# microsoft/EVA

Hardware: AMD Instinct MI355X
Metric: homomorphic ops/sec (mul+rescale+relin) at N=2^16, L=10; execute() wall-time (higher is better)
Workload: dtype u64

## Files before the change

### eva_amd/backend.py

```python
import ctypes as C
import os

import numpy as np

from . import _hipruntime

_HERE = os.path.dirname(os.path.abspath(__file__))
LIB_PATH = os.path.join(_HERE, "lib", "libeva_hip.so")

KEY_RELIN = 0
KEY_GALOIS = 1
F64, F32, U8 = 0, 1, 2
_DTYPES = {np.dtype(np.float64): F64, np.dtype(np.float32): F32, np.dtype(np.uint8): U8}


def array_dtype(a):
    a = np.asarray(a)
    if a.dtype not in _DTYPES or not a.flags["C_CONTIGUOUS"]:
        a = np.ascontiguousarray(a, dtype=np.float64)
    return a, _DTYPES[a.dtype]


class EvaHipError(RuntimeError):
    pass
# ... 8 lines not shown
    "evah_ctx_create": [C.c_uint32, C.c_uint32, _u64p, C.c_int, _vpp],
    "evah_ctx_fork": [_vp, _vpp],
    "evah_ctx_set_stream": [_vp, _vp],
    "evah_ctx_sync": [_vp],
    "evah_ctx_mem_info": [_vp, C.POINTER(C.c_size_t), C.POINTER(C.c_size_t)],
    "evah_key_upload": [_vp, C.c_int, C.c_uint32, C.c_uint32, _u64p],
    "evah_galois_elt_from_step": [_vp, C.c_int32, C.POINTER(C.c_uint32)],
    "evah_ct_upload": [_vp, C.c_uint32, C.c_uint32, C.c_double, _u64p, _vpp],
    "evah_ct_write": [_vp, _vp, _u64p],
    "evah_ct_copy": [_vp, _vp, _vpp],
    "evah_ct_assign": [_vp, _vp, _vp],
    "evah_ctx_wait": [_vp, _vp],
    "evah_ctx_transfer_stats": [_vp, _u64p],
    "evah_ctx_modup_variant": [_vp, C.POINTER(C.c_uint32)],
    "evah_ctx_tail_variant": [_vp, C.POINTER(C.c_uint32)],
    "evah_ctx_key_bytes": [_vp, _u64p],
    "evah_ctx_key_bytes_detail": [_vp, _u64p],
    "evah_ctx_key_upload_stats": [_vp, _u64p],
    "evah_pt_copy": [_vp, _vp, _vpp],
    "evah_pt_write": [_vp, _vp, _u64p],
    "evah_capture_begin": [_vp, _vpp, C.c_uint32],
    "evah_capture_end": [_vp, _vpp, C.c_uint32, _vpp],
    "evah_graph_launch": [_vp, _vp],
    "evah_ct_info": [_vp, C.POINTER(C.c_uint32), C.POINTER(C.c_uint32), C.POINTER(C.c_double)],
    "evah_ct_download": [_vp, _vp, _u64p],
    "evah_pt_upload": [_vp, C.c_uint32, C.c_double, _u64p, _vpp],
    "evah_pt_upload_coeff": [_vp, C.c_uint32, C.c_double, _u64p, _vpp],
    "evah_pt_uniform": [_vp, C.c_uint32, C.c_double, _u64p, _vpp],
    "evah_pt_info": [_vp, C.POINTER(C.c_uint32), C.POINTER(C.c_double)],
    "evah_pt_download": [_vp, _vp, _u64p],
# ... 639 lines not shown
    def transfer_stats(self):
        out = (C.c_uint64 * 6)()
        _chk(_lib.evah_ctx_transfer_stats(self.h, out))
        return tuple(int(x) for x in out)

    def modup_variant(self):
        out = (C.c_uint32 * 3)()
        _chk(_lib.evah_ctx_modup_variant(self.h, out))
        return int(out[0]), bool(out[1]), bool(out[2])

    def tail_variant(self):
        out = (C.c_uint32 * 3)()
        _chk(_lib.evah_ctx_tail_variant(self.h, out))
        return bool(out[0]), bool(out[1]), bool(out[2])

    def key_bytes(self):
        out = C.c_uint64()
        _chk(_lib.evah_ctx_key_bytes(self.h, C.byref(out)))
        return int(out.value)

    def key_bytes_detail(self):
        out = (C.c_uint64 * 3)()
        _chk(_lib.evah_ctx_key_bytes_detail(self.h, out))
        return tuple(int(x) for x in out)

    def key_upload_stats(self):
        out = (C.c_uint64 * 2)()
        _chk(_lib.evah_ctx_key_upload_stats(self.h, out))
        return tuple(int(x) for x in out)

# ... 376 lines not shown
```

### eva_amd/csrc/internal.hip.h

```cpp
#pragma once
#include "../../include/eva_hip.h"

#include <hip/hip_runtime.h>

#include <algorithm>
#include <cmath>
#include <cstdlib>
#include <cstring>
#include <functional>
#include <map>
#include <memory>
#include <mutex>
#include <stdexcept>
#include <string>
#include <tuple>
#include <unordered_map>
#include <vector>

#include "devmath.hip.h"
#include "hostmath.h"

namespace evah {

extern thread_local std::string g_err;
// ... 183 lines not shown
  bool fold_pa = true;
  bool win_fuse = true;
  bool win_linear = true;
  bool fb_persist = true;
  uint32_t fb_grid = 0;
  bool mac3 = true;
  uint32_t loop_n = 8, loop_min = 2, loop_min_wgs = 2048, loop_target_wgs = 8192;
  bool hoist_map = true;
  bool side_stream = false;
  bool chain_step = true, chain_batched = true;
  uint32_t chain_fuse_blocks = 256;
  bool modup = true;
  int modup_lr = 3;
  bool modup_spec = true;
  bool tail_fuse = true;
  uint32_t lds_extra = 0;
  uint32_t keygen_set_words = 1u << 27;

  static Tunables from_env(uint32_t N) {
    Tunables t;
    auto flag = [](const char *name, bool &v) { if (const char *e = std::getenv(name)) v = std::atoi(e) != 0; };
    auto count = [](const char *name, uint32_t &v) { if (const char *e = std::getenv(name)) v = (uint32_t)std::max(0, std::atoi(e)); };
    (void)N;
    flag("EVAH_FUSE_MAC", t.fuse_mac);
    flag("EVAH_FUSE_MUL", t.fuse_mul);
    flag("EVAH_FUSE_MUL2", t.fuse_mul2);
    flag("EVAH_EW_FUSE", t.ew_fuse);
    flag("EVAH_EW_UNIFORM", t.ew_uniform);
    count("EVAH_FUSE_SMALL", t.fuse_small_blocks);
    if (const char *e = std::getenv("EVAH_SMALL_LR")) t.small_lr = std::atoi(e) == 3 ? 3 : 2;
// ... 13 lines not shown
    count("EVAH_LOOP_N", t.loop_n);
    count("EVAH_LOOP_MIN", t.loop_min);
    count("EVAH_LOOP_MIN_WGS", t.loop_min_wgs);
    count("EVAH_LOOP_TARGET_WGS", t.loop_target_wgs);
    count("EVAH_LDS_EXTRA", t.lds_extra);
    count("EVAH_KEYGEN_SET_WORDS", t.keygen_set_words);
    flag("EVAH_HOIST_MAP", t.hoist_map);
    flag("EVAH_SIDE_STREAM", t.side_stream);
    flag("EVAH_CHAIN_STEP", t.chain_step);
    flag("EVAH_CHAIN_BATCHED", t.chain_batched);
    count("EVAH_CHAIN_FUSE_BLOCKS", t.chain_fuse_blocks);
    flag("EVAH_MODUP", t.modup);
    if (const char *e = std::getenv("EVAH_MODUP_LR")) t.modup_lr = std::atoi(e) == 2 ? 2 : 3;
    flag("EVAH_MODUP_SPEC", t.modup_spec);
    flag("EVAH_TAIL_FUSE", t.tail_fuse);
    if (const char *e = std::getenv("EVAH_KS_GROUPS")) t.ks_groups = std::max(1, std::atoi(e));
    if (const char *e = std::getenv("EVAH_KS_THREADS")) {
      const int n = std::atoi(e);
      if (n == 64 || n == 128 || n == 256) t.ks_threads = n;
    }
    return t;
  }
};

struct evah_ctx {
  std::shared_ptr<SharedDev> sh;
  int device = 0;
  uint32_t N = 0, logN = 0, k = 0;
  std::vector<u64> primes;
  std::vector<int> total_bits;
// ... 25 lines not shown

#ifndef EVAH_TOPBIT
#define EVAH_TOPBIT 1
#endif
struct ModupVariant { int lr; bool tbonly, lazyonly; };
inline ModupVariant modup_variant(const evah_ctx *c) {
  const bool tb = c->tun.modup_spec && EVAH_TOPBIT && c->modup_tb;
  return {c->tun.modup_lr, tb, tb && c->modup_lazy};
}
struct TailVariant { bool fused, tbonly, lazyonly; };
inline TailVariant tail_variant(const evah_ctx *c) {
  const bool tb = c->tun.modup_spec && EVAH_TOPBIT && c->modup_tb;
  return {c->tun.tail_fuse, tb, tb && c->tail_lazy};
}

inline void use(evah_ctx *c) { HIPCHK(hipSetDevice(c->device)); }
inline void count_h2d(evah_ctx *c, size_t bytes, bool plain = false) { c->sh->xfer[plain ? 2 : 0]++; c->sh->xfer[4] += bytes; }
inline void count_d2h(evah_ctx *c, size_t bytes, bool plain = false) { c->sh->xfer[plain ? 3 : 1]++; c->sh->xfer[5] += bytes; }

inline hipEvent_t prof_event(evah_ctx *c) {
  if (!c->prof_free.empty()) {
    hipEvent_t e = c->prof_free.back();
    c->prof_free.pop_back();
    return e;
  }
  hipEvent_t e;
  HIPCHK(hipEventCreate(&e));
  return e;
}
inline void prof_drain(evah_ctx *c) {
// ... 259 lines not shown
```

### eva_amd/csrc/keyswitch.hip

```cpp
#include "launch.hip.h"

namespace evah {

__global__ void __launch_bounds__(256)
k_ks_mac(DevCtx cx, const u64 *target, const u64 *scratch, const u64 *key, u64 *prod, uint32_t l) {
  if (cx.skipped()) return;
  const uint32_t I = blockIdx.y;
  const uint32_t kap = (I == l) ? cx.k - 1 : I;
  const size_t n = 2 * ((size_t)blockIdx.x * blockDim.x + threadIdx.x);
  const DevPrime pm = cx.primes[kap];
  const size_t N = cx.N, key_digit = (size_t)2 * cx.k * N;
  u128_t a0x = {0, 0}, a0y = {0, 0}, a1x = {0, 0}, a1y = {0, 0};
  for (uint32_t J = 0; J < l; J++) {
    const u64 *op = (I == J) ? target + (size_t)J * N : scratch + ((size_t)I * l + J) * N;
    const ulonglong2 o = ld2(op + n);
    const u64 *kp = key + J * key_digit + (size_t)kap * N + n;
    const ulonglong2 k0 = ld2(kp), k1 = ld2(kp + (size_t)cx.k * N);
    acc128(a0x, o.x, k0.x);
    acc128(a0y, o.y, k0.y);
    acc128(a1x, o.x, k1.x);
    acc128(a1y, o.y, k1.y);
  }
  ulonglong2 r0, r1;
  r0.x = barrett128(a0x, pm);
// ... 24 lines not shown
  return kb;
}

template <int P>
static void launch_ks_inner_p(evah_ctx *c, const u64 *target, const u64 *scratch, const KsBatch &kb, u64 *prod, uint32_t l) {
  constexpr int LR = KS_LR;
  ProfScope ps(c, KC_KSMAC);
  const uint32_t tile = ks_wg_threads(c) << LR;
  const bool one_wave = ks_one_wave(c);
  const int logC = (int)ilog2(tile) - P;
  if (logC < 0) throw std::runtime_error("ks_inner tile smaller than one sub-transform");
  const size_t lds = ((((size_t)1 << logC) * lds_sub_stride<P>() + 1) & ~(size_t)1) * sizeof(u64) +
                     ((size_t)1 << (logC + P)) * sizeof(ulonglong2) +
                     (kb.mac3 ? (size_t)tile * sizeof(u64) : 0);
  const uint32_t n_tiles = c->N / tile;
  auto go = [&](auto kernel, const auto &mt, const auto &at) {
    hipLaunchKernelGGL(kernel, dim3(n_tiles * kb.n, kb.ni), dim3(tile >> LR), lds, c->stream, c->dev, target, kb.target_bs, scratch,
                       kb.scratch_bs, kb.keys, prod, kb.prod_bs, l, kb.i0, logC, n_tiles, kb.n, kb.targets, mt, kb.istep,
                       kb.nout ? kb.nout : l + 1, kb.r_out, at, (kb.lazy_out ? 1 : 0) | (kb.diag ? 2 : 0), kb.fold_row);
  };
  if (kb.r_out && (!one_wave || kb.istep != 1)) throw std::logic_error("fused special-row inverse pass needs the one-wave key-switch kernel");
  if (kb.fold && kb.istep != 1) throw std::logic_error("the folded key-switch forms are not used on limb shards");
  if (kb.fold && !kb.mul && !kb.adds) throw std::logic_error("folded key switch without polynomials to fold");
  const int mode = kb.mul ? (kb.fold ? KS_FOLDMUL : KS_MUL) : (kb.fold ? KS_FOLDADD : KS_PLAIN);
  auto with_mode = [&](auto mode_tag) {
    constexpr int M = decltype(mode_tag)::value;
    const KsMulArg<M> mt = [&] { if constexpr (M == KS_MUL || M == KS_FOLDMUL) return *kb.mul; else return NoMul{}; }();
    const KsAddArg<M> at = [&] { if constexpr (M == KS_FOLDADD) return *kb.adds; else return NoMul{}; }();
    if constexpr (M != KS_MUL) {
      if (kb.mac3 && one_wave) {
        if (kb.r_out) go(ks_inner_kernel<P, LR, 64, M, true, true>, mt, at);
        else go(ks_inner_kernel<P, LR, 64, M, false, true>, mt, at);
        return;
      }
    }
    if (kb.mac3) throw std::logic_error("split keys handed to a key-switch kernel that accumulates in 128 bits");
    if (kb.r_out) go(ks_inner_kernel<P, LR, 64, M, true>, mt, at);
    else if (one_wave) go(ks_inner_kernel<P, LR, 64, M>, mt, at);
    else go(ks_inner_kernel<P, LR, NTT_THREADS, M>, mt, at);
  };
  switch (mode) {
  case KS_PLAIN: with_mode(std::integral_constant<int, KS_PLAIN>{}); break;
  case KS_MUL: with_mode(std::integral_constant<int, KS_MUL>{}); break;
// ... 7 lines not shown
  case 5: launch_ks_inner_p<5>(c, target, scratch, key, prod, l); break;
  case 6: launch_ks_inner_p<6>(c, target, scratch, key, prod, l); break;
  case 7: launch_ks_inner_p<7>(c, target, scratch, key, prod, l); break;
  case 8: launch_ks_inner_p<8>(c, target, scratch, key, prod, l); break;
  default: throw std::runtime_error("unsupported poly_modulus_degree for the key-switch kernel");
  }
}

static bool ks_small(evah_ctx *c, uint32_t l, uint32_t n) {
  return c->tun.fuse_mac && std::max(1, c->tun.ks_groups) == 1 && fuse_small_launch(c, n * (l + 1) * l);
}
static bool ks_takes_modup(evah_ctx *c, uint32_t l, uint32_t n) {
  return !ks_small(c, l, n) && c->tun.modup && c->tun.fuse_mac && std::max(1, c->tun.ks_groups) == 1 && modup_fits(c);
}

bool switch_key_products(evah_ctx *c, uint32_t l, const u64 *target, size_t target_bs, const KeyDev *const *keys,
                         uint32_t n, u64 *prod_d, const PtrTab *target_tab, const MulTab *mul, u64 *r_small, bool fold,
                         const PtrTab *adds, bool lazy_out) {
  const size_t N = c->N;
  KsBatch kb = ks_batch(c, l, keys, n, !(mul && !fold));
  kb.target_bs = target_bs;
  if (target_tab) kb.targets = *target_tab;
  kb.mul = mul;
  kb.fold = fold;
  kb.adds = adds;
  kb.lazy_out = lazy_out;
  if ((mul || fold) && !c->tun.fuse_mac) throw std::logic_error("the fused multiply / folded forms need the fused key-switch kernel");
  Scratch t(c, (size_t)n * l * N);
  Scratch sc(c, n * kb.scratch_bs);
  Scratch d2(c, mul && fold ? (size_t)n * l * N : 1);
  if (mul && fold) {
    target = d2.d;
    kb.target_bs = target_bs = (size_t)l * N;
  }
  OpKsDigit::Params dp{t.d, sc.d, l, (size_t)l * N, kb.scratch_bs, 0, l + 1};
// ... 9 lines not shown
    if (small || modup) launch_pass_p<false, true, OpPlain>(c, c->logN / 2, ip, n * l);
    else ntt_inverse<OpPlain>(c, ip, n * l);
  }
  if (small) {
    dp.i0 = kb.i0 = 0;
    dp.ni = kb.ni = l + 1;
    launch_inv_fwd<OpKsDigit>(c, dp, n * (l + 1) * l);
    if (r_small && c->tun.fuse_special_inv && ks_one_wave(c)) kb.r_out = r_small;
    launch_ks_inner(c, c->logN / 2, target, sc.d, kb, prod_d, l);
    return kb.r_out != nullptr;
  }
  if (c->tun.fuse_mac) {
    const int a = (c->logN + 1) / 2, b = c->logN / 2;
    const uint32_t groups = std::min<uint32_t>(std::max(1, c->tun.ks_groups), l + 1);
    if (r_small && groups == 1 && c->tun.fuse_special_inv && ks_one_wave(c)) kb.r_out = r_small;
    for (uint32_t g = 0; g < groups; g++) {
      const uint32_t i0 = (uint32_t)((uint64_t)(l + 1) * g / groups), i1 = (uint32_t)((uint64_t)(l + 1) * (g + 1) / groups);
      if (i1 == i0) continue;
      dp.i0 = kb.i0 = i0;
      dp.ni = kb.ni = i1 - i0;
      if (modup) launch_modup<OpKsDigit>(c, dp, n);
      else launch_pass_p<true, false, OpKsDigit>(c, a, dp, n * (i1 - i0) * l);
      launch_ks_inner(c, b, target, sc.d, kb, prod_d, l);
    }
    return kb.r_out != nullptr;
  } else {
    ntt_forward<OpKsDigit>(c, dp, n * (l + 1) * l);
    for (uint32_t b = 0; b < n; b++) {
      ProfScope ps(c, KC_KSMAC);
      hipLaunchKernelGGL(k_ks_mac, dim3(c->N / 512, l + 1), dim3(256), 0, c->stream, c->dev,
// ... 62 lines not shown
  OpModDown::Params mp{r.d, N, prod.d, pps, nullptr, 0, 0, out_d, (size_t)l * N, c->k - 1, l};
  mp.use_add_tab = !fold;
  mp.add_tab = in.c01;
  inverse_then_forward<OpPlain, OpModDown>(c, sp, 2 * n, mp, 2 * n * l, inv1);
}

static void relin_rescale_core(evah_ctx *c, uint32_t l, uint32_t n, const Size3Tab *in, const MulTab *mul, u64 *out_d) {
  const uint32_t last = l - 1, sp = c->k - 1;
  const size_t N = c->N, pps = (size_t)(l + 1) * N, ops = (size_t)(l - 1) * N;
  PtrTab c2{}, a_last{}, a_polys{};
  if (in) {
    c2 = in->c2;
    a_polys = in->c01;
    for (uint32_t i = 0; i < 2 * n; i++) a_last.p[i] = a_polys.p[i] + (size_t)last * N;
  }
  Scratch prod(c, (size_t)n * 2 * pps);
  std::vector<const KeyDev *> keys(n, &c->sh->relin);
  const bool fold = c->tun.fold_pa && c->tun.fuse_mac;
  switch_key_products(c, l, nullptr, 0, keys.data(), n, prod.d, &c2, mul, nullptr, fold, mul ? nullptr : &a_polys, fold);
  Scratch r(c, (size_t)n * 2 * N), t(c, (size_t)n * 2 * N);
  if (fold && tail_variant(c).fused && ks_takes_modup(c, l, n)) {
    OpRRLastFolded::Params lp{nullptr, 0, prod.d + (size_t)last * N, pps, r.d, N, t.d, N, last, sp, {}};
    OpTailIntt::Params ip{lp, prod.d + (size_t)l * N, pps, r.d};
    launch_pass_p<false, true, OpTailIntt>(c, c->logN / 2, ip, 4 * n);
    OpRRFolded::Params rp{r.d, N, t.d, N, nullptr, 0, prod.d, pps, out_d, ops, sp, last, l - 1, {}};
    launch_tail(c, lp, rp, 2 * n);
    launch_pass_p<false, false, OpRRFolded>(c, c->logN / 2, rp, 2 * n * (l - 1));
    return;
  }
  OpPlain::Params spp{prod.d + (size_t)l * N, r.d, pps, N, 1, sp, 1, {}};
  ntt_inverse<OpPlain>(c, spp, 2 * n);
  if (fold) {
    OpRRLastFolded::Params lp{nullptr, 0, prod.d + (size_t)last * N, pps, r.d, N, t.d, N, last, sp, {}};
// ... 335 lines not shown
```

### eva_amd/csrc/launch.hip.h

```cpp
#pragma once
#include "internal.hip.h"
#include "ntt.hip.h"

namespace evah {

#define EW_SETUP                                                                                 \
  const uint32_t p = blockIdx.z, i = blockIdx.y;                                                 \
  const size_t off = (size_t)i * cx.N + 2 * ((size_t)blockIdx.x * blockDim.x + threadIdx.x);    \
  const DevPrime pm = cx.primes[cx.prime_of(i)];                                                 \
  (void)p;                                                                                        \
  (void)pm;

__device__ __forceinline__ ulonglong2 ld2(const u64 *p) { return *reinterpret_cast<const ulonglong2 *>(p); }
__device__ __forceinline__ void st2(u64 *p, ulonglong2 v) { *reinterpret_cast<ulonglong2 *>(p) = v; }
__device__ __forceinline__ u64 split30(u64 k) { return (k & 0x3fffffffull) | ((k >> 30) << 32); }

template <class Op> struct OpClass;
template <bool Z, bool G> struct OpClass<OpPlainT<Z, G>> { static constexpr int fwd_a = KC_NTT_A, fwd_b = KC_NTT_B; };
template <> struct OpClass<OpMulIntt> { static constexpr int fwd_a = KC_NTT_A, fwd_b = KC_NTT_B; };
template <> struct OpClass<OpKsDigit> { static constexpr int fwd_a = KC_KSDIGIT_A, fwd_b = KC_KSDIGIT_B; };
template <bool G> struct OpClass<OpModDownT<G>> { static constexpr int fwd_a = KC_MODDOWN_A, fwd_b = KC_MODDOWN_B; };
template <> struct OpClass<OpMulPolyIntt> { static constexpr int fwd_a = KC_NTT_A, fwd_b = KC_NTT_B; };
template <> struct OpClass<OpModDownMul> { static constexpr int fwd_a = KC_MODDOWN_A, fwd_b = KC_MODDOWN_B; };
template <int M> struct OpClass<OpRRT<M>> { static constexpr int fwd_a = KC_MODDOWN_A, fwd_b = KC_MODDOWN_B; };
// ... 91 lines not shown
struct KsBatch {
  uint32_t n = 1;
  uint32_t i0 = 0, ni = 0;
  size_t target_bs = 0, scratch_bs = 0, prod_bs = 0;
  KsKeys keys{};
  PtrTab targets{};
  const MulTab *mul = nullptr;
  bool fold = false;
  const PtrTab *adds = nullptr;
  bool mac3 = false;
  bool lazy_out = false;
  uint32_t istep = 1, nout = 0;
  u64 *r_out = nullptr;
  bool diag = false;
  uint32_t fold_row = ~0u;
};
inline std::vector<double> fill_mul_tab(evah_ctx *c, const evah_ct *const *as, const evah_ct *const *bs, uint32_t pairs, uint32_t B,
                                        uint32_t l, const char *batch_msg, MulTab &tab) {
  std::vector<double> scales(pairs);
  for (uint32_t i = 0; i < pairs; i++) {
    const evah_ct *a = as[i], *b = bs[i];
    if (a->size != 2 || b->size != 2) throw std::invalid_argument("multiply supports size-2 operands only (relinearize first)");
    if (a->batch != B || b->batch != B) throw std::invalid_argument(batch_msg);
    if (a->limbs != l || b->limbs != l) throw std::invalid_argument("encrypted parameter mismatch in batch");
    scales[i] = a->scale * b->scale;
    check_scale(c, scales[i], l);
    acquire(c, a->buf);
    acquire(c, b->buf);
    for (uint32_t x = 0; x < B; x++) {
      tab.a[i * B + x] = a->d + (size_t)x * 2 * a->ps;
// ... 135 lines not shown
static void inverse_then_forward(evah_ctx *c, const typename InvOp::Params &ip, uint32_t inv_jobs, const typename Op::Params &fp,
                                 uint32_t fwd_jobs, bool inv_pass1_done = false) {
  if (inv_pass1_done && !fuse_small_launch(c, fwd_jobs)) throw std::logic_error("fused inverse pass outside the small-launch form");
  if (fuse_small_launch(c, fwd_jobs)) {
    if (!inv_pass1_done) launch_pass_p<false, true, InvOp>(c, c->logN / 2, ip, inv_jobs);
    launch_inv_fwd<Op>(c, fp, fwd_jobs);
    launch_pass_p<false, false, Op>(c, c->logN / 2, fp, fwd_jobs);
  } else {
    ntt_inverse<InvOp>(c, ip, inv_jobs);
    ntt_forward<Op>(c, fp, fwd_jobs);
  }
}

bool switch_key_products(evah_ctx *c, uint32_t l, const u64 *target, size_t target_bs, const KeyDev *const *keys, uint32_t n,
                         u64 *prod_d, const PtrTab *target_tab = nullptr, const MulTab *mul = nullptr, u64 *r_small = nullptr,
                         bool fold = false, const PtrTab *adds = nullptr, bool lazy_out = false);
void switch_key(evah_ctx *c, uint32_t l, const u64 *target, const KeyDev &key, const u64 *add, size_t add_ps, uint32_t add_polys,
                u64 *out, size_t out_ps);
void key_split_launch(evah_ctx *c, const u64 *src, u64 *dst, size_t words);
const uint32_t *perm_table(evah_ctx *c, uint32_t elt);
void galois_perm_launch(evah_ctx *c, const u64 *a, size_t a_ps, uint32_t limbs, uint32_t polys, const uint32_t *perm, u64 *out, size_t o_ps);
void enc_tables(evah_ctx *c);

}
```

### eva_amd/csrc/ntt_ks_inner.hip.h

```cpp
#pragma once
#include "ntt.hip.h"

namespace evah {

#ifndef EVAH_KS_BATCH_MAX_DEFINED
#define EVAH_KS_BATCH_MAX_DEFINED
constexpr int KS_BATCH_MAX = 64;
#endif
struct KsKeys {
  const u64 *key[KS_BATCH_MAX];
  uint32_t rows;
};
struct PtrTab {
  const u64 *p[2 * KS_BATCH_MAX];
};

struct MulTab {
  const u64 *a[KS_BATCH_MAX], *b[KS_BATCH_MAX];
  uint32_t a_ps[KS_BATCH_MAX], b_ps[KS_BATCH_MAX];
};
struct MulSrc {
  const u64 *a, *b;
  size_t sa, sb;
};
// ... 34 lines not shown
  s2 = mad64(v1, (uint32_t)(kw >> 32), s2);
}
__device__ __forceinline__ void mac3_fold(u64 &s0, u64 &s1, u64 &s2) {
  s1 += s0 >> 30;
  s0 &= 0x3fffffffull;
  s2 += s1 >> 30;
  s1 &= 0x3fffffffull;
}
__device__ __forceinline__ u128_t mac3_recombine(u64 s0, u64 s1, u64 s2) {
  unsigned __int128 a = s0;
  a += (unsigned __int128)s1 << 30;
  a += (unsigned __int128)s2 << 60;
  return {(u64)a, (u64)(a >> 64)};
}

template <int P, int LR, int MAXT, int MODE, bool INVSP = false, bool MAC3 = false>
__global__ void __launch_bounds__(MAXT)
ks_inner_kernel(DevCtx cx, const u64 *__restrict__ target_b, size_t target_bs, const u64 *__restrict__ scratch_b,
                size_t scratch_bs, KsKeys keys, u64 *__restrict__ prod_b, size_t prod_bs, uint32_t l, uint32_t i0,
                int logC, uint32_t n_tiles, uint32_t n_inst, PtrTab targets, KsMulArg<MODE> mul, uint32_t istep,
                uint32_t nout, u64 *__restrict__ r_out, KsAddArg<MODE> adds, int flags, uint32_t fold_row) {
  const bool lazy_out = flags & 1, diag = flags & 2;
  constexpr bool MUL = MODE == KS_MUL;
  extern __shared__ __attribute__((aligned(16))) u64 lds[];
  if (cx.skipped()) return;
  uint32_t tile_idx, inst;
  if ((n_tiles & 7u) == 0) {
    const uint32_t x = blockIdx.x, lo = x & 7u, rest = x >> 3;
    inst = rest % n_inst;
    tile_idx = (rest / n_inst) * 8u + lo;
  } else {
    inst = blockIdx.x / n_tiles;
    tile_idx = blockIdx.x % n_tiles;
  }
  inst = __builtin_amdgcn_readfirstlane(inst);
  tile_idx = __builtin_amdgcn_readfirstlane(tile_idx);
// ... 174 lines not shown
    if (++since_fold == KS128_FOLD_DIGITS && J + 1 < l) {
      since_fold = 0;
#pragma unroll
      for (int i = 0; i < NTT_R; i++) {
        ks128_fold(acc0[i], pm);
        ks128_fold(acc1[i], pm);
      }
    }
  }
  if constexpr (MAC3) {
#pragma unroll
    for (int i = 0; i < NTT_R; i++) {
      acc0[i] = mac3_recombine(s0[0][i], s1[0][i], s2[0][i]);
      acc1[i] = mac3_recombine(s0[1][i], s1[1][i], s2[1][i]);
    }
  }
  if constexpr (MODE == KS_FOLDMUL || MODE == KS_FOLDADD) {
    {
      const ulonglong2 Pm = (fold_row != ~0u) ? cx.plinv[(size_t)fold_row * cx.k + kap]
                                                                     : cx.modq[(size_t)(cx.k - 1) * cx.k + kap];
      const size_t off = (size_t)(Irow < l ? Irow : l - 1) * N + gbase;
#pragma unroll
      for (int it = 0; it < NPAIR; it++) {
        const size_t o = off + 2 * (threadIdx.x + it * T);
        if constexpr (MODE == KS_FOLDMUL) {
          const ulonglong2 a0 = *reinterpret_cast<const ulonglong2 *>(msrc.a + o);
          const ulonglong2 a1 = *reinterpret_cast<const ulonglong2 *>(msrc.a + msrc.sa + o);
          const ulonglong2 b0 = *reinterpret_cast<const ulonglong2 *>(msrc.b + o);
          const ulonglong2 b1 = *reinterpret_cast<const ulonglong2 *>(msrc.b + msrc.sb + o);
          const u64 u0x = mul_tw_lazy5(b0.x, Pm.x, Pm.y, pm.nq), u0y = mul_tw_lazy5(b0.y, Pm.x, Pm.y, pm.nq);
// ... 38 lines not shown
        __syncthreads();
        u64 *r = r_out + ((size_t)2 * inst + K) * N + gbase;
#pragma unroll
        for (int it = 0; it < NPAIR; it++) {
          const int idx = 2 * (threadIdx.x + it * T);
          const int sb = idx >> P, e = idx & (S - 1);
          ulonglong2 v;
          v.x = lds[sb * SP + lds_pad<P>(e)];
          v.y = lds[sb * SP + lds_pad<P>(e + 1)];
          *reinterpret_cast<ulonglong2 *>(r + idx) = v;
        }
      }
      return;
    }
  }
  u64 *p0 = prod + (size_t)Irow * N + gbase, *p1 = prod + ((size_t)nout + Irow) * N + gbase;
  if (lazy_out && I != l) {
#pragma unroll
    for (int it = 0; it < NPAIR; it++) {
      const int idx = 2 * (threadIdx.x + it * T);
      ulonglong2 r0, r1;
      r0.x = reduce128_lazy(acc0[2 * it], pm);
      r0.y = reduce128_lazy(acc0[2 * it + 1], pm);
      r1.x = reduce128_lazy(acc1[2 * it], pm);
      r1.y = reduce128_lazy(acc1[2 * it + 1], pm);
      *reinterpret_cast<ulonglong2 *>(p0 + idx) = r0;
      *reinterpret_cast<ulonglong2 *>(p1 + idx) = r1;
    }
    return;
  }
// ... 15 lines not shown
```

### eva_amd/csrc/ntt_ops.hip.h

```cpp
#pragma once
#include "ntt.hip.h"
#include "ntt_window_sum.hip.h"
#include "ntt_ks_inner.hip.h"

namespace evah {


struct NoGather {};
template <bool ZEROS, bool GATHER = false> struct OpPlainT {
  struct Params {
    const u64 *src;
    u64 *dst;
    size_t src_ps, dst_ps;
    uint32_t jl, prime0;
    int addhalf;
    PtrTab src_tab;
    uint32_t pstep = 1;
    u64 *zero_list = nullptr;
    std::conditional_t<GATHER, PermTab, NoGather> perm_tab{};
    u64 *clear_base = nullptr;
    uint32_t clear_words = 0;
  };
  static constexpr bool clears_words = ZEROS;
  struct Job {
// ... 422 lines not shown
    j.pinv = cx.invq[p.sp * cx.k + i];
    j.linv = cx.invq[p.last * cx.k + i];
    j.lazy = cx.primes[p.last].q <= cx.primes[i].q4 && cx.primes[p.sp].q <= cx.primes[i].q8;
    return true;
  }
  template <bool LZ> static __device__ __forceinline__ u64 conv(const Job &j, const DevPrime &pm, u64 r, u64 t) {
    if (LZ) return mul_tw_lazy5(r + (pm.q - j.halfP), j.pinv.x, j.pinv.y, pm.nq) + (t + (pm.q - j.halfL));
    const u64 u = submod(barrett64(r, pm.q, pm.brt), j.halfP, pm.q);
    const u64 v = submod(barrett64(t, pm.q, pm.brt), j.halfL, pm.q);
    return addmod(mul_shoup(u, j.pinv.x, j.pinv.y, pm.q), v, pm.q);
  }
  template <bool LZ>
  static __device__ __forceinline__ u64 load(const DevCtx &, const Job &j, const DevPrime &pm, uint32_t n) {
    return conv<LZ>(j, pm, j.r[n], j.t[n]);
  }
  static __device__ __forceinline__ void store_fwd(const DevCtx &cx, const Job &j, const DevPrime &pm, uint32_t n, u64 W) {
    W += (W >= pm.q8 ? pm.nq8 : 0);
    u64 av = 0;
    if constexpr (AM != RR_FOLDED) av = MUL ? product_poly(j.mul, j.K, j.off + n, pm) : j.a[n];
    const u64 x = av + mul_tw_lazy5(j.prod[n], j.pinv.x, j.pinv.y, pm.nq) + pm.q8 - W;
    j.dst[n] = mul_shoup(x, j.linv.x, j.linv.y, pm.q);
  }
  struct LoopPre { u64 prod, a; };
  static __device__ __forceinline__ LoopPre loop_prefetch(const DevCtx &, const Job &j, const DevPrime &, uint32_t n) {
    return LoopPre{j.prod[n], AM == RR_MEM ? j.a[n] : 0};
  }
  static __device__ __forceinline__ void store_fwd_loop(const DevCtx &cx, const Job &j, const DevPrime &pm, uint32_t n, u64 W, const LoopPre &p) {
    if constexpr (AM == RR_MUL) {
      store_fwd(cx, j, pm, n, W);
    } else {
      W += (W >= pm.q8 ? pm.nq8 : 0);
      const u64 x = p.a + mul_tw_lazy5(p.prod, j.pinv.x, j.pinv.y, pm.nq) + pm.q8 - W;
      j.dst[n] = mul_shoup(x, j.linv.x, j.linv.y, pm.q);
    }
  }
};

using OpRRLast = OpRRLastT<RR_MEM>;
using OpRRLastMul = OpRRLastT<RR_MUL>;
using OpRRLastFolded = OpRRLastT<RR_FOLDED>;
using OpRR = OpRRT<RR_MEM>;
using OpRRMul = OpRRT<RR_MUL>;
using OpRRFolded = OpRRT<RR_FOLDED>;

struct OpTailIntt {
  using Last = OpRRLastT<RR_FOLDED>;
  struct Params {
    Last::Params lp;
// ... 32 lines not shown
```

### eva_amd/csrc/runtime.hip

```cpp
#include "internal.hip.h"
namespace evah {
void key_split_launch(evah_ctx *c, const u64 *src, u64 *dst, size_t words);
void ct_stack_launch(evah_ctx *c, const evah_ct *const *cts, uint32_t n, evah_ct *o);
}

namespace evah {

thread_local std::string g_err;

static std::mutex g_ctx_mu;
static std::vector<const void *> g_live_ctx;
void ctx_register(const void *c) {
  std::lock_guard<std::mutex> lk(g_ctx_mu);
  g_live_ctx.push_back(c);
}
void ctx_unregister(const void *c) {
  std::lock_guard<std::mutex> lk(g_ctx_mu);
  g_live_ctx.erase(std::remove(g_live_ctx.begin(), g_live_ctx.end(), c), g_live_ctx.end());
}
bool ctx_alive(const void *c) {
  std::lock_guard<std::mutex> lk(g_ctx_mu);
  return std::find(g_live_ctx.begin(), g_live_ctx.end(), c) != g_live_ctx.end();
}

// ... 628 lines not shown
  out[0] = (uint32_t)v.lr;
  out[1] = v.tbonly;
  out[2] = v.lazyonly;
  API_END
}

int evah_ctx_tail_variant(evah_ctx *c, uint32_t out[3]) {
  API_BEGIN
  const TailVariant v = tail_variant(c);
  out[0] = v.fused;
  out[1] = v.tbonly;
  out[2] = v.lazyonly;
  API_END
}

int evah_ctx_transfer_stats(evah_ctx *c, uint64_t out[6]) {
  API_BEGIN
  for (int i = 0; i < 6; i++) out[i] = c->sh->xfer[i];
  API_END
}

int evah_ctx_key_bytes(evah_ctx *c, uint64_t *bytes) {
  API_BEGIN
  uint64_t b = c->sh->relin.d ? c->sh->relin.bytes : 0;
  for (auto &kv : c->sh->galois) b += kv.second.bytes;
  *bytes = b;
  API_END
}

int evah_ctx_key_upload_stats(evah_ctx *c, uint64_t out[2]) {
// ... 257 lines not shown
```

### include/eva_hip.h

```cpp
#ifndef EVA_HIP_H
#define EVA_HIP_H
#include <stddef.h>
#include <stdint.h>

#ifdef __cplusplus
extern "C" {
#endif

typedef struct evah_ctx evah_ctx;
typedef struct evah_ct evah_ct;
typedef struct evah_pt evah_pt;
typedef struct evah_graph evah_graph;

const char *evah_last_error(void);
int evah_abi_version(void);
int evah_device_count(int *count);

int evah_ctx_create(uint32_t poly_degree, uint32_t n_primes, const uint64_t *primes, int device,
                    evah_ctx **out);
int evah_ctx_fork(evah_ctx *parent, evah_ctx **out);
void evah_ctx_destroy(evah_ctx *ctx);
int evah_ctx_set_stream(evah_ctx *ctx, void *hip_stream);
int evah_ctx_sync(evah_ctx *ctx);
int evah_ctx_busy(evah_ctx *ctx, int *busy);
// ... 35 lines not shown
int evah_ct_download_instances_async(evah_ctx *ctx, const evah_ct *ct, uint64_t *const *out);
int evah_ct_batch(const evah_ct *ct, uint32_t *batch);
int evah_ct_stack(evah_ctx *ctx, const evah_ct *const *cts, uint32_t n, evah_ct **out);
int evah_ct_unstack(evah_ctx *ctx, const evah_ct *ct, uint32_t b, evah_ct **out);
int evah_ct_slice(evah_ctx *ctx, const evah_ct *ct, uint32_t b0, uint32_t n, evah_ct **out);

int evah_ct_copy(evah_ctx *dst_ctx, const evah_ct *src, evah_ct **out);
int evah_pt_copy(evah_ctx *dst_ctx, const evah_pt *src, evah_pt **out);
int evah_ct_write(evah_ctx *ctx, evah_ct *ct, const uint64_t *data);
int evah_pt_write(evah_ctx *ctx, evah_pt *pt, const uint64_t *data);
int evah_ct_assign(evah_ctx *ctx, evah_ct *dst, const evah_ct *src);
int evah_ctx_wait(evah_ctx *waiter, evah_ctx *signaller);
int evah_ctx_transfer_stats(evah_ctx *ctx, uint64_t out[6]);
int evah_ctx_modup_variant(evah_ctx *ctx, uint32_t out[3]);
int evah_ctx_tail_variant(evah_ctx *ctx, uint32_t out[3]);
int evah_ctx_key_bytes(evah_ctx *ctx, uint64_t *bytes);
int evah_ctx_key_bytes_detail(evah_ctx *ctx, uint64_t out[3]);
int evah_ctx_key_upload_stats(evah_ctx *ctx, uint64_t out[2]);
int evah_ctx_stack_stats(evah_ctx *ctx, uint64_t out[2]);
int evah_ct_info(const evah_ct *ct, uint32_t *size, uint32_t *limbs, double *scale);
int evah_ct_download(evah_ctx *ctx, const evah_ct *ct, uint64_t *out );
void evah_ct_free(evah_ctx *ctx, evah_ct *ct);
int evah_pt_upload(evah_ctx *ctx, uint32_t limbs, double scale, const uint64_t *data ,
                   evah_pt **out);
int evah_pt_upload_coeff(evah_ctx *ctx, uint32_t limbs, double scale, const uint64_t *data,
                         evah_pt **out);
int evah_pt_encode(evah_ctx *ctx, const double *values, uint32_t n_values, uint32_t limbs, double scale, evah_pt **out);
int evah_pt_uniform(evah_ctx *ctx, uint32_t limbs, double scale, const uint64_t *value ,
                    evah_pt **out);
int evah_pt_info(const evah_pt *pt, uint32_t *limbs, double *scale);
// ... 146 lines not shown
```

Before: 15800.

## Fuse rescale tail epilogue into key-switch inner kernel for relinearization

Adds two epilogue variants to the one-wave folded key-switch kernel. Variant A writes the special-prime and last-limb rows through an inverse NTT directly. Variant B combines the remaining rows with the forward-NTT correction loaded via global-to-LDS DMA and writes the final output, so the intermediate product buffer and a separate rescale-tail pass are no longer needed. It is gated by a heuristic on the workgroup count and on several tunables, and exposes a query API. The cost is more complex kernels, possible register pressure, and a serialized A to tail to B launch order.

```diff
diff --git a/eva_amd/backend.py b/eva_amd/backend.py
--- a/eva_amd/backend.py
+++ b/eva_amd/backend.py
@@ -46,6 +46,7 @@
     "evah_ctx_transfer_stats": [_vp, _u64p],
     "evah_ctx_modup_variant": [_vp, C.POINTER(C.c_uint32)],
     "evah_ctx_tail_variant": [_vp, C.POINTER(C.c_uint32)],
+    "evah_ctx_ks_tail": [_vp, C.POINTER(C.c_uint32)],
     "evah_ctx_key_bytes": [_vp, _u64p],
     "evah_ctx_key_bytes_detail": [_vp, _u64p],
     "evah_ctx_key_upload_stats": [_vp, _u64p],
@@ -715,6 +716,11 @@
         _chk(_lib.evah_ctx_tail_variant(self.h, out))
         return bool(out[0]), bool(out[1]), bool(out[2])
 
+    def ks_tail(self):
+        out = (C.c_uint32 * 2)()
+        _chk(_lib.evah_ctx_ks_tail(self.h, out))
+        return bool(out[0]), int(out[1])
+
     def key_bytes(self):
         out = C.c_uint64()
         _chk(_lib.evah_ctx_key_bytes(self.h, C.byref(out)))
diff --git a/eva_amd/csrc/internal.hip.h b/eva_amd/csrc/internal.hip.h
--- a/eva_amd/csrc/internal.hip.h
+++ b/eva_amd/csrc/internal.hip.h
@@ -221,6 +221,8 @@
   int modup_lr = 3;
   bool modup_spec = true;
   bool tail_fuse = true;
+  int ks_tail = -1;
+  uint32_t ks_tail_min_wgs = 4096;
   uint32_t lds_extra = 0;
   uint32_t keygen_set_words = 1u << 27;
 
@@ -264,6 +266,8 @@
     if (const char *e = std::getenv("EVAH_MODUP_LR")) t.modup_lr = std::atoi(e) == 2 ? 2 : 3;
     flag("EVAH_MODUP_SPEC", t.modup_spec);
     flag("EVAH_TAIL_FUSE", t.tail_fuse);
+    if (const char *e = std::getenv("EVAH_KS_TAIL")) t.ks_tail = std::atoi(e) != 0 ? 1 : 0;
+    count("EVAH_KS_TAIL_MIN_WGS", t.ks_tail_min_wgs);
     if (const char *e = std::getenv("EVAH_KS_GROUPS")) t.ks_groups = std::max(1, std::atoi(e));
     if (const char *e = std::getenv("EVAH_KS_THREADS")) {
       const int n = std::atoi(e);
@@ -319,6 +323,15 @@
   return {c->tun.tail_fuse, tb, tb && c->tail_lazy};
 }
 
+struct KsTailVariant { bool on; uint32_t min_wgs; };
+inline KsTailVariant ks_tail_variant(const evah_ctx *c) {
+  const bool one_wave = (std::min<uint32_t>(c->N, (uint32_t)c->tun.ks_threads << 2) >> 2) <= 64;
+  const bool modup = c->tun.modup && std::max(1, c->tun.ks_groups) == 1 && c->N >= 2048 && (c->logN + 1) / 2 <= 9;
+  const bool on = c->tun.ks_tail != 0 && c->tun.fold_pa && c->tun.fuse_mac && c->tun.tail_fuse && modup && EVAH_TOPBIT &&
+                  c->modup_tb && c->tun.mac3 && c->all_tb && one_wave;
+  return {on, on && c->tun.ks_tail < 0 ? c->tun.ks_tail_min_wgs : 0};
+}
+
 inline void use(evah_ctx *c) { HIPCHK(hipSetDevice(c->device)); }
 inline void count_h2d(evah_ctx *c, size_t bytes, bool plain = false) { c->sh->xfer[plain ? 2 : 0]++; c->sh->xfer[4] += bytes; }
 inline void count_d2h(evah_ctx *c, size_t bytes, bool plain = false) { c->sh->xfer[plain ? 3 : 1]++; c->sh->xfer[5] += bytes; }
diff --git a/eva_amd/csrc/keyswitch.hip b/eva_amd/csrc/keyswitch.hip
--- a/eva_amd/csrc/keyswitch.hip
+++ b/eva_amd/csrc/keyswitch.hip
@@ -62,19 +62,29 @@
                      ((size_t)1 << (logC + P)) * sizeof(ulonglong2) +
                      (kb.mac3 ? (size_t)tile * sizeof(u64) : 0);
   const uint32_t n_tiles = c->N / tile;
-  auto go = [&](auto kernel, const auto &mt, const auto &at) {
+  auto go_tail = [&](auto kernel, const auto &mt, const auto &at, const auto &tl) {
     hipLaunchKernelGGL(kernel, dim3(n_tiles * kb.n, kb.ni), dim3(tile >> LR), lds, c->stream, c->dev, target, kb.target_bs, scratch,
                        kb.scratch_bs, kb.keys, prod, kb.prod_bs, l, kb.i0, logC, n_tiles, kb.n, kb.targets, mt, kb.istep,
-                       kb.nout ? kb.nout : l + 1, kb.r_out, at, (kb.lazy_out ? 1 : 0) | (kb.diag ? 2 : 0), kb.fold_row);
+                       kb.nout ? kb.nout : l + 1, kb.r_out, at, (kb.lazy_out ? 1 : 0) | (kb.diag ? 2 : 0), kb.fold_row, tl);
   };
-  if (kb.r_out && (!one_wave || kb.istep != 1)) throw std::logic_error("fused special-row inverse pass needs the one-wave key-switch kernel");
+  auto go = [&](auto kernel, const auto &mt, const auto &at) { go_tail(kernel, mt, at, NoMul{}); };
+  if (kb.r_out && !kb.tail && (!one_wave || kb.istep != 1)) throw std::logic_error("fused special-row inverse pass needs the one-wave key-switch kernel");
   if (kb.fold && kb.istep != 1) throw std::logic_error("the folded key-switch forms are not used on limb shards");
   if (kb.fold && !kb.mul && !kb.adds) throw std::logic_error("folded key switch without polynomials to fold");
+  if (kb.tail) {
+    const bool rows_ok = kb.tail == KS_TAIL_A ? (kb.i0 + 1 == l && kb.ni == 2 && kb.tail_out.t) : (kb.i0 == 0 && kb.ni + 1 == l && kb.tail_out.dst_ps);
+    if (P < 6 || !kb.mac3 || !one_wave || !kb.fold || kb.istep != 1 || kb.diag || kb.fold_row != ~0u || !kb.r_out || l < 2 || !rows_ok)
+      throw std::logic_error("key-switch tail epilogue outside its form");
+  }
   const int mode = kb.mul ? (kb.fold ? KS_FOLDMUL : KS_MUL) : (kb.fold ? KS_FOLDADD : KS_PLAIN);
   auto with_mode = [&](auto mode_tag) {
     constexpr int M = decltype(mode_tag)::value;
     const KsMulArg<M> mt = [&] { if constexpr (M == KS_MUL || M == KS_FOLDMUL) return *kb.mul; else return NoMul{}; }();
     const KsAddArg<M> at = [&] { if constexpr (M == KS_FOLDADD) return *kb.adds; else return NoMul{}; }();
+    if constexpr ((M == KS_FOLDMUL || M == KS_FOLDADD) && P >= 6) {
+      if (kb.tail == KS_TAIL_A) { go_tail(ks_inner_kernel<P, LR, 64, M, false, true, KS_TAIL_A>, mt, at, kb.tail_out); return; }
+      if (kb.tail == KS_TAIL_B) { go_tail(ks_inner_kernel<P, LR, 64, M, false, true, KS_TAIL_B>, mt, at, kb.tail_out); return; }
+    }
     if constexpr (M != KS_MUL) {
       if (kb.mac3 && one_wave) {
         if (kb.r_out) go(ks_inner_kernel<P, LR, 64, M, true, true>, mt, at);
@@ -112,11 +122,19 @@
   return !ks_small(c, l, n) && c->tun.modup && c->tun.fuse_mac && std::max(1, c->tun.ks_groups) == 1 && modup_fits(c);
 }
 
+static bool ks_tail_applies(evah_ctx *c, uint32_t l, uint32_t n) {
+  const KsTailVariant v = ks_tail_variant(c);
+  if (!v.on || l < 2 || !ks_takes_modup(c, l, n) || !ks_mac3(c, l)) return false;
+  if (!c->sh->relin.d_split || c->sh->relin.rows != c->k || c->sh->relin.n_digits < l) return false;
+  return (uint64_t)2 * n * (c->N / 256) >= v.min_wgs;
+}
+
 bool switch_key_products(evah_ctx *c, uint32_t l, const u64 *target, size_t target_bs, const KeyDev *const *keys,
                          uint32_t n, u64 *prod_d, const PtrTab *target_tab, const MulTab *mul, u64 *r_small, bool fold,
-                         const PtrTab *adds, bool lazy_out) {
+                         const PtrTab *adds, bool lazy_out, const KsTailPlan *tail) {
   const size_t N = c->N;
   KsBatch kb = ks_batch(c, l, keys, n, !(mul && !fold));
+  if (tail && !(kb.mac3 && fold && ks_takes_modup(c, l, n))) throw std::logic_error("key-switch tail epilogue outside its form");
   kb.target_bs = target_bs;
   if (target_tab) kb.targets = *target_tab;
   kb.mul = mul;
@@ -156,6 +174,25 @@
     const int a = (c->logN + 1) / 2, b = c->logN / 2;
     const uint32_t groups = std::min<uint32_t>(std::max(1, c->tun.ks_groups), l + 1);
     if (r_small && groups == 1 && c->tun.fuse_special_inv && ks_one_wave(c)) kb.r_out = r_small;
+    if (tail) {
+      dp.i0 = 0;
+      dp.ni = l + 1;
+      launch_modup<OpKsDigit>(c, dp, n);
+      kb.tail = KS_TAIL_A;
+      kb.i0 = l - 1;
+      kb.ni = 2;
+      kb.r_out = const_cast<u64 *>(tail->lp.r);
+      kb.tail_out = KsTailOut{tail->lp.t, 0};
+      launch_ks_inner(c, b, target, sc.d, kb, nullptr, l);
+      launch_tail(c, tail->lp, tail->rp, 2 * n);
+      kb.tail = KS_TAIL_B;
+      kb.i0 = 0;
+      kb.ni = l - 1;
+      kb.r_out = tail->rp.dst;
+      kb.tail_out = KsTailOut{nullptr, tail->rp.dst_ps};
+      launch_ks_inner(c, b, target, sc.d, kb, nullptr, l);
+      return false;
+    }
     for (uint32_t g = 0; g < groups; g++) {
       const uint32_t i0 = (uint32_t)((uint64_t)(l + 1) * g / groups), i1 = (uint32_t)((uint64_t)(l + 1) * (g + 1) / groups);
       if (i1 == i0) continue;
@@ -248,9 +285,16 @@
     a_polys = in->c01;
     for (uint32_t i = 0; i < 2 * n; i++) a_last.p[i] = a_polys.p[i] + (size_t)last * N;
   }
-  Scratch prod(c, (size_t)n * 2 * pps);
   std::vector<const KeyDev *> keys(n, &c->sh->relin);
   const bool fold = c->tun.fold_pa && c->tun.fuse_mac;
+  if (ks_tail_applies(c, l, n)) {
+    Scratch r(c, (size_t)n * 2 * N), t(c, (size_t)n * 2 * N);
+    KsTailPlan plan{OpRRLastFolded::Params{nullptr, 0, nullptr, pps, r.d, N, t.d, N, last, sp, {}},
+                    OpRRFolded::Params{r.d, N, t.d, N, nullptr, 0, nullptr, pps, out_d, ops, sp, last, l - 1, {}}};
+    switch_key_products(c, l, nullptr, 0, keys.data(), n, nullptr, &c2, mul, nullptr, fold, mul ? nullptr : &a_polys, true, &plan);
+    return;
+  }
+  Scratch prod(c, (size_t)n * 2 * pps);
   switch_key_products(c, l, nullptr, 0, keys.data(), n, prod.d, &c2, mul, nullptr, fold, mul ? nullptr : &a_polys, fold);
   Scratch r(c, (size_t)n * 2 * N), t(c, (size_t)n * 2 * N);
   if (fold && tail_variant(c).fused && ks_takes_modup(c, l, n)) {
diff --git a/eva_amd/csrc/launch.hip.h b/eva_amd/csrc/launch.hip.h
--- a/eva_amd/csrc/launch.hip.h
+++ b/eva_amd/csrc/launch.hip.h
@@ -129,6 +129,12 @@
   u64 *r_out = nullptr;
   bool diag = false;
   uint32_t fold_row = ~0u;
+  int tail = KS_TAIL_NONE;
+  KsTailOut tail_out{};
+};
+struct KsTailPlan {
+  OpRRLastFolded::Params lp;
+  OpRRFolded::Params rp;
 };
 inline std::vector<double> fill_mul_tab(evah_ctx *c, const evah_ct *const *as, const evah_ct *const *bs, uint32_t pairs, uint32_t B,
                                         uint32_t l, const char *batch_msg, MulTab &tab) {
@@ -294,7 +300,7 @@
 
 bool switch_key_products(evah_ctx *c, uint32_t l, const u64 *target, size_t target_bs, const KeyDev *const *keys, uint32_t n,
                          u64 *prod_d, const PtrTab *target_tab = nullptr, const MulTab *mul = nullptr, u64 *r_small = nullptr,
-                         bool fold = false, const PtrTab *adds = nullptr, bool lazy_out = false);
+                         bool fold = false, const PtrTab *adds = nullptr, bool lazy_out = false, const KsTailPlan *tail = nullptr);
 void switch_key(evah_ctx *c, uint32_t l, const u64 *target, const KeyDev &key, const u64 *add, size_t add_ps, uint32_t add_polys,
                 u64 *out, size_t out_ps);
 void key_split_launch(evah_ctx *c, const u64 *src, u64 *dst, size_t words);
diff --git a/eva_amd/csrc/ntt_ks_inner.hip.h b/eva_amd/csrc/ntt_ks_inner.hip.h
--- a/eva_amd/csrc/ntt_ks_inner.hip.h
+++ b/eva_amd/csrc/ntt_ks_inner.hip.h
@@ -72,12 +72,26 @@
   return {(u64)a, (u64)(a >> 64)};
 }
 
-template <int P, int LR, int MAXT, int MODE, bool INVSP = false, bool MAC3 = false>
+constexpr int KS_TAIL_NONE = 0, KS_TAIL_A = 1, KS_TAIL_B = 2;
+struct KsTailOut {
+  u64 *t;
+  size_t dst_ps;
+};
+template <int TAIL> struct KsTailArgs { using Out = KsTailOut; };
+template <> struct KsTailArgs<KS_TAIL_NONE> { using Out = NoMul; };
+template <int TAIL> using KsTailArg = typename KsTailArgs<TAIL>::Out;
+template <int AM> struct OpRRT;
+template <int TAIL> struct KsTailOps { using RR = OpRRT<2>; };
+
+template <int P, int LR, int MAXT, int MODE, bool INVSP = false, bool MAC3 = false, int TAIL = KS_TAIL_NONE>
 __global__ void __launch_bounds__(MAXT)
 ks_inner_kernel(DevCtx cx, const u64 *__restrict__ target_b, size_t target_bs, const u64 *__restrict__ scratch_b,
                 size_t scratch_bs, KsKeys keys, u64 *__restrict__ prod_b, size_t prod_bs, uint32_t l, uint32_t i0,
                 int logC, uint32_t n_tiles, uint32_t n_inst, PtrTab targets, KsMulArg<MODE> mul, uint32_t istep,
-                uint32_t nout, u64 *__restrict__ r_out, KsAddArg<MODE> adds, int flags, uint32_t fold_row) {
+                uint32_t nout, u64 *__restrict__ r_out, KsAddArg<MODE> adds, int flags, uint32_t fold_row,
+                KsTailArg<TAIL> tail) {
+  static_assert(TAIL == KS_TAIL_NONE || (MAC3 && !INVSP && MAXT == 64 && (MODE == KS_FOLDMUL || MODE == KS_FOLDADD)),
+                "the tail epilogues belong to the one-wave radix-2^30 kernel in a fold mode");
   const bool lazy_out = flags & 1, diag = flags & 2;
   constexpr bool MUL = MODE == KS_MUL;
   extern __shared__ __attribute__((aligned(16))) u64 lds[];
@@ -282,6 +296,19 @@
       acc0[i] = mac3_recombine(s0[0][i], s1[0][i], s2[0][i]);
       acc1[i] = mac3_recombine(s0[1][i], s1[1][i], s2[1][i]);
     }
+  }
+  u64 *tail_row = nullptr;
+  size_t tail_ps = 0;
+  auto dma_corr = [&](int K) {
+    asm volatile("s_waitcnt lgkmcnt(0)" ::: "memory");
+#pragma unroll
+    for (int it = 0; it < NPAIR; it++)
+      __builtin_amdgcn_global_load_lds(tail_row + (size_t)K * tail_ps + 2 * (threadIdx.x + it * T), lin + 2 * it * T, 16, 0, 0);
+  };
+  if constexpr (TAIL == KS_TAIL_B) {
+    tail_ps = tail.dst_ps;
+    tail_row = r_out + (size_t)2 * inst * tail_ps + (size_t)I * N + gbase;
+    dma_corr(0);
   }
   if constexpr (MODE == KS_FOLDMUL || MODE == KS_FOLDADD) {
     {
@@ -350,6 +377,95 @@
       return;
     }
   }
+  if constexpr (TAIL == KS_TAIL_A) {
+    const bool special = I == l;
+    const ulonglong2 *twi = cx.tw_inv + (size_t)kap * cx.N;
+    const ulonglong2 pinv = cx.invq[(size_t)(cx.k - 1) * cx.k + kap];
+    __syncthreads();
+    for (int idx = threadIdx.x; idx < (C << P); idx += T) {
+      const int sb = idx >> P, n = idx & (S - 1);
+      if (n) {
+        const int d = 31 - __clz(n);
+        twl[idx] = twi[((size_t)((1u << pre) + sub0 + sb) << d) + (n - (1 << d))];
+      }
+    }
+#pragma unroll
+    for (int K = 0; K < 2; K++) {
+      __syncthreads();
+#pragma unroll
+      for (int it = 0; it < NPAIR; it++) {
+        const int idx = 2 * (threadIdx.x + it * T);
+        const int sb = idx >> P, e = idx & (S - 1);
+        const u128_t ax = K ? acc1[2 * it] : acc0[2 * it], ay = K ? acc1[2 * it + 1] : acc0[2 * it + 1];
+        u64 vx, vy;
+        if (special) {
+          vx = barrett128(ax, pm);
+          vy = barrett128(ay, pm);
+        } else {
+          vx = mul_shoup(reduce128_lazy(ax, pm), pinv.x, pinv.y, pm.q);
+          vy = mul_shoup(reduce128_lazy(ay, pm), pinv.x, pinv.y, pm.q);
+        }
+        lds[sb * SP + lds_pad<P>(e)] = vx;
+        lds[sb * SP + lds_pad<P>(e + 1)] = vy;
+      }
+      __syncthreads();
+      RoundSeq<P, LR, 0, true, true, true, false>::run(lds + sub * SP, tid, 0, 0, twl + (sub << P), pm);
+      __syncthreads();
+      u64 *r = (special ? r_out : tail.t) + ((size_t)2 * inst + K) * N + gbase;
+#pragma unroll
+      for (int it = 0; it < NPAIR; it++) {
+        const int idx = 2 * (threadIdx.x + it * T);
+        const int sb = idx >> P, e = idx & (S - 1);
+        ulonglong2 v;
+        v.x = lds[sb * SP + lds_pad<P>(e)];
+        v.y = lds[sb * SP + lds_pad<P>(e + 1)];
+        *reinterpret_cast<ulonglong2 *>(r + idx) = v;
+      }
+    }
+    return;
+  }
+  if constexpr (TAIL == KS_TAIL_B) {
+    using RR = typename KsTailOps<TAIL>::RR;
+    using RS = Rounds<P, LR>;
+    const ulonglong2 pinv = cx.invq[(size_t)(cx.k - 1) * cx.k + kap], linv = cx.invq[(size_t)(l - 1) * cx.k + kap];
+    u64 red[2][NTT_R];
+#pragma unroll
+    for (int i = 0; i < NTT_R; i++) {
+      red[0][i] = reduce128_lazy(acc0[i], pm);
+      red[1][i] = reduce128_lazy(acc1[i], pm);
+    }
+#pragma unroll
+    for (int K = 0; K < 2; K++) {
+      asm volatile("s_waitcnt vmcnt(0)" ::: "memory");
+      __builtin_amdgcn_wave_barrier();
+      auto next_tile = [&]() { if (K == 0) dma_corr(1); };
+      ntt_round<P, LR, RS::bits(0), RS::lo(0), false, true, true, true, true>(lds + sub * SP, tid, 0, 0, twl + (sub << P), pm,
+                                                                            lin + sub * S, next_tile);
+      if constexpr (RS::NR > 1) {
+        __builtin_amdgcn_wave_barrier();
+        RoundSeq<P, LR, 1, false, true, true, true, true, true>::run(lds + sub * SP, tid, 0, 0, twl + (sub << P), pm);
+      }
+      __builtin_amdgcn_wave_barrier();
+      const __amdgpu_buffer_rsrc_t out = __builtin_amdgcn_make_buffer_rsrc(tail_row + (size_t)K * tail_ps, 0, 0x7fffffff, 0x00020000);
+#pragma unroll
+      for (int it = 0; it < NPAIR; it++) {
+        const int idx = 2 * (threadIdx.x + it * T);
+        const int sb = idx >> P, e = idx & (S - 1);
+        const u64 wx = lds[sb * SP + lds_pad<P>(e)], wy = lds[sb * SP + lds_pad<P>(e + 1)];
+        ulonglong2 v;
+        v.x = RR::combine(pm, pinv, linv, 0, red[K][2 * it], wx);
+        v.y = RR::combine(pm, pinv, linv, 0, red[K][2 * it + 1], wy);
+        typedef unsigned int u32x4 __attribute__((ext_vector_type(4)));
+        u32x4 w;
+        w.x = (uint32_t)v.x;
+        w.y = (uint32_t)(v.x >> 32);
+        w.z = (uint32_t)v.y;
+        w.w = (uint32_t)(v.y >> 32);
+        __builtin_amdgcn_raw_buffer_store_b128(w, out, 16u * threadIdx.x + 16u * (uint32_t)(it * T), 0, 0);
+      }
+    }
+    return;
+  }
   u64 *p0 = prod + (size_t)Irow * N + gbase, *p1 = prod + ((size_t)nout + Irow) * N + gbase;
   if (lazy_out && I != l) {
 #pragma unroll
diff --git a/eva_amd/csrc/ntt_ops.hip.h b/eva_amd/csrc/ntt_ops.hip.h
--- a/eva_amd/csrc/ntt_ops.hip.h
+++ b/eva_amd/csrc/ntt_ops.hip.h
@@ -460,12 +460,15 @@
   static __device__ __forceinline__ u64 load(const DevCtx &, const Job &j, const DevPrime &pm, uint32_t n) {
     return conv<LZ>(j, pm, j.r[n], j.t[n]);
   }
+  static __device__ __forceinline__ u64 combine(const DevPrime &pm, ulonglong2 pinv, ulonglong2 linv, u64 av, u64 prod, u64 W) {
+    W += (W >= pm.q8 ? pm.nq8 : 0);
+    const u64 x = av + mul_tw_lazy5(prod, pinv.x, pinv.y, pm.nq) + pm.q8 - W;
+    return mul_shoup(x, linv.x, linv.y, pm.q);
+  }
   static __device__ __forceinline__ void store_fwd(const DevCtx &cx, const Job &j, const DevPrime &pm, uint32_t n, u64 W) {
-    W += (W >= pm.q8 ? pm.nq8 : 0);
     u64 av = 0;
     if constexpr (AM != RR_FOLDED) av = MUL ? product_poly(j.mul, j.K, j.off + n, pm) : j.a[n];
-    const u64 x = av + mul_tw_lazy5(j.prod[n], j.pinv.x, j.pinv.y, pm.nq) + pm.q8 - W;
-    j.dst[n] = mul_shoup(x, j.linv.x, j.linv.y, pm.q);
+    j.dst[n] = combine(pm, j.pinv, j.linv, av, j.prod[n], W);
   }
   struct LoopPre { u64 prod, a; };
   static __device__ __forceinline__ LoopPre loop_prefetch(const DevCtx &, const Job &j, const DevPrime &, uint32_t n) {
@@ -475,9 +478,7 @@
     if constexpr (AM == RR_MUL) {
       store_fwd(cx, j, pm, n, W);
     } else {
-      W += (W >= pm.q8 ? pm.nq8 : 0);
-      const u64 x = p.a + mul_tw_lazy5(p.prod, j.pinv.x, j.pinv.y, pm.nq) + pm.q8 - W;
-      j.dst[n] = mul_shoup(x, j.linv.x, j.linv.y, pm.q);
+      j.dst[n] = combine(pm, j.pinv, j.linv, p.a, p.prod, W);
     }
   }
 };
diff --git a/eva_amd/csrc/runtime.hip b/eva_amd/csrc/runtime.hip
--- a/eva_amd/csrc/runtime.hip
+++ b/eva_amd/csrc/runtime.hip
@@ -666,6 +666,14 @@
   API_END
 }
 
+int evah_ctx_ks_tail(evah_ctx *c, uint32_t out[2]) {
+  API_BEGIN
+  const KsTailVariant v = ks_tail_variant(c);
+  out[0] = v.on;
+  out[1] = v.min_wgs;
+  API_END
+}
+
 int evah_ctx_transfer_stats(evah_ctx *c, uint64_t out[6]) {
   API_BEGIN
   for (int i = 0; i < 6; i++) out[i] = c->sh->xfer[i];
diff --git a/include/eva_hip.h b/include/eva_hip.h
--- a/include/eva_hip.h
+++ b/include/eva_hip.h
@@ -73,6 +73,7 @@
 int evah_ctx_transfer_stats(evah_ctx *ctx, uint64_t out[6]);
 int evah_ctx_modup_variant(evah_ctx *ctx, uint32_t out[3]);
 int evah_ctx_tail_variant(evah_ctx *ctx, uint32_t out[3]);
+int evah_ctx_ks_tail(evah_ctx *ctx, uint32_t out[2]);
 int evah_ctx_key_bytes(evah_ctx *ctx, uint64_t *bytes);
 int evah_ctx_key_bytes_detail(evah_ctx *ctx, uint64_t out[3]);
 int evah_ctx_key_upload_stats(evah_ctx *ctx, uint64_t out[2]);
```

Result: faster. 16510, median of 6 (+4.5%).
